# s-will/BiAlign

Hardware: AMD Instinct MI355X
Metric: giga-DP-cells/sec (higher is better)
Workload: dtype int32

## Files before the change

### bialign_amd/csrc/bialign_fill_slim.hpp

```cpp
#pragma once

namespace bialign {

template <int S, int TW, int PPW, bool LEAN = false>
__global__ void __launch_bounds__(64 * TW * PPW, 3) fill_affine_slim_kernel(const DeviceBatch A) {
  static_assert(S >= 1, "packed records need a band");
  using PK_ = Pack<S>;
  using G_ = Geo<S>;
  using R_ = Rec<S, 9, LEAN>;
  constexpr int W = G_::W, R = G_::R, RR = G_::RR, PADB = G_::PADB;
  constexpr int ND = R_::ND, NCH4 = R_::NCH4, TAIL = R_::TAIL, RECDW = R_::RECDW;
  static_assert(R * W < 64, "lane 63 must be free: it is the sentinel source of the exchange");
  extern __shared__ __align__(16) int32_t smem[];

  constexpr int T = TW;
  constexpr int NW = TW * PPW;
  const int L = threadIdx.x & 63;
  const int wv = NW == 1 ? 0 : __builtin_amdgcn_readfirstlane(threadIdx.x >> 6);
  const int pw = wv / TW, w = wv - pw * TW;
  const int slot = blockIdx.x * PPW + pw;
  const bool have_pair = slot < A.launch_pairs;
  const int pid = A.order[have_pair ? slot : 0];
  const PairDesc pd = A.pairs[pid];
  const int n = pd.n, m = pd.m, P = pd.P;
  const int il = L / W, aa = L - il * W;
  const bool live = L < R * W;
  const bool ghost = (il == 0);
  int ringfed_v = (ghost || !live) ? 1 : 0;
  asm volatile("" : "+v"(ringfed_v));
  const bool ringfed = ringfed_v != 0;
  int storing_v;
  {
    const int pad_idx0 = L < W ? L : (L >= R * W ? W + (L - R * W) : 64);
    storing_v = ((live && (LEAN ? il == R - 1 : !ghost)) || (!LEAN && pad_idx0 < R_::SLP - R_::SL)) ? 1 : 0;
  }
  asm volatile("" : "+v"(storing_v));
  const bool storing = storing_v != 0;
  const int beta = A.beta, gamma = A.gamma, delta = A.delta;
  const int k1 = A.k1, k2 = A.k2;
  const int gD = gamma + delta, gg = 2 * gamma, ggdd = 2 * gamma + 2 * delta, dd = 2 * delta;

  using GF = GhostFeed<S, 9, LEAN, 0>;
  constexpr int PERW = GF::RING_DW;
  constexpr int SENTBLK = 4 * GF::NP;
  v4i* ring = reinterpret_cast<v4i*>(smem + wv * GF::RING_DW);
  int32_t* sentblk = smem + NW * PERW;
  volatile int32_t* prog_lds = smem + NW * PERW + SENTBLK + pw * TW;
  const volatile int32_t* const fit_floor = smem + NW * PERW + SENTBLK + FIT_FLOOR_WORD;
  const volatile int32_t* const col0_floor = smem + NW * PERW + SENTBLK + COL0_FLOOR_WORD;
  int32_t* offtab = smem + NW * PERW + SENTBLK + LDS_PROG_WORDS;
  int32_t* s1 = offtab + slim_offtab_dw<S>();
  int32_t* s2 = s1 + k1 * k1;
  uint8_t* codes = reinterpret_cast<uint8_t*>(s2 + k2 * k2);
  const int npad = code_pad(n), mpad = code_pad(m, PADB);
  uint8_t* sa = codes + (size_t)pw * A.slim_code_bytes;
  uint8_t* ca = sa + npad;
  uint8_t* sb = ca + npad;
  uint8_t* cb = sb + mpad;

  for (int t = threadIdx.x; t < NW * PERW + SENTBLK; t += 64 * NW) smem[t] = SENT;
  if (threadIdx.x < LDS_PROG_WORDS) smem[NW * PERW + SENTBLK + threadIdx.x] = prog_word_init(threadIdx.x, A.free_ends);
  if (!LEAN)
    for (int t = threadIdx.x; t < GF::OFFTAB_DW; t += 64 * NW) offtab[t] = (int32_t)GF::lane_offset(t >> 6, t & 63);
  for (int t = threadIdx.x; t < k1 * k1; t += 64 * NW) s1[t] = A.s1[t];
  for (int t = threadIdx.x; t < k2 * k2; t += 64 * NW) s2[t] = A.s2[t];
  if (have_pair) {
    const int tt = threadIdx.x - pw * (64 * TW);
    for (int t = tt; t < n; t += 64 * TW) {
      sa[t] = A.seq_a[pd.seq_a + t];
      ca[t] = A.cls_a[pd.seq_a + t];
    }
    for (int t = tt; t < m + 2 * PADB; t += 64 * TW) {
      const int src = t - PADB;
      const bool ok = src >= 0 && src < m;
      sb[t] = ok ? A.seq_b[pd.seq_b + src] : 0;
      cb[t] = ok ? A.cls_b[pd.seq_b + src] : 0;
    }
  }
  __syncthreads();
  if (!have_pair) return;

  const int addrA = ((L - W) & 63) * 4;
  const int addrB = (live && aa < W - 1 ? ((L - W + 1) & 63) : 63) * 4;
  const bool a_first = (aa == 0);
  const int lane_cap = a_first ? SENT : 0x7fffffff;
  int32_t* const lay = A.layers + pd.layer_off;
  const int64_t pk_bnd_off = (int64_t)pd.G * PK_::RECDW;
  const int rec_last = pd.G - 1;
  const int NSw = (pd.NS - w + T - 1) / T;
  const int H = NSw > 0 ? (NSw - 1) * P + m + G_::MAXOFF + 1 : 0;

  int jj = -(2 * il + aa);
  int strip = 0;
  int rec_base = w * P;
  int i = 0, s1row = 0, s2row = 0;
  bool act_row = false;
  auto set_row = [&](int q) {
    i = (q * T + w) * RR + il - 1;
    const int k = i + aa - S;
    act_row = live && i >= 0 && i <= n && k >= 0 && k <= n;
    s1row = (i >= 1 && i <= n) ? sa[i - 1] * k1 : 0;
    s2row = (k >= 1 && k <= n) ? ca[k - 1] * k2 : 0;
  };
  set_row(0);

  int dA1[2][W], dA2[2][W];
  int dAx[2][W];
  int dB[4][W];
  int dC[2][W];
  int selfv[4][W];
  int pubC[W][8];
  int inC[W][8];
  int inA[W][4], inB[W][8];
#pragma unroll
  for (int bb = 0; bb < W; ++bb) {
    dA1[0][bb] = dA1[1][bb] = dA2[0][bb] = dA2[1][bb] = SENT;
    dAx[0][bb] = dAx[1][bb] = dC[0][bb] = dC[1][bb] = SENT;
#pragma unroll
    for (int x = 0; x < 4; ++x) dB[x][bb] = selfv[x][bb] = inA[bb][x] = SENT;
#pragma unroll
    for (int x = 0; x < 8; ++x) pubC[bb][x] = inB[bb][x] = inC[bb][x] = SENT;
  }
  const uint32_t ring_lds = __builtin_amdgcn_readfirstlane(
      (uint32_t)(uintptr_t)(__attribute__((address_space(3))) int32_t*)smem) + wv * GF::RING_DW * 4;

  using SA = StepAddr<S, LEAN>;
  using GS = GhostSrc<S, LEAN>;
  typedef const __attribute__((address_space(3))) int32_t* lds_cptr;
  typedef __attribute__((address_space(1))) char* gbl_ptr;
  typedef __attribute__((address_space(1))) v4i* gbl_v4i;
  typedef __attribute__((address_space(1))) int32_t* gbl_i32;
  uint32_t st_off = SA::chunk_off(L), st_toff = SA::tail_off(L), gs_fac = GS::factor(L);
  uint32_t gs_lane = GS::lane_byte(L, ring_lds + (NW - wv) * GF::RING_DW * 4);
  asm volatile("" : "+v"(st_off), "+v"(st_toff), "+v"(gs_fac), "+v"(gs_lane));
  int s_ph = 0, s_q = 0;
  int s_adv = 0;
  uint32_t ring_u = 0;
  gbl_ptr sbase = nullptr;

  int blk_q = 0, blk_rem = 0;
  int seen_prog = -0x40000000;
  auto wait_partner = [&](int h_last) __attribute__((always_inline)) {
    if (T == 1) return;
    const int src = w == 0 ? T - 1 : w - 1;
    const int need = h_last + 2 * (R - 1) + 1 - (w == 0 ? P : 0);
    if (seen_prog >= need) return;
    for (int spin = 0; (seen_prog = prog_lds[src]) < need; ++spin) {
      if (spin > A.spin_limit) {
        if (L == 0) atomicOr(A.errflag, 1);
        seen_prog = 0x7fffffff;
        break;
      }
      __builtin_amdgcn_s_sleep(16);
    }
  };
  bool blk_steady = false;
  auto prefetch_block = [&](int h0, int half) __attribute__((always_inline)) {
    wait_partner(h0 + GF::BLK - 1);
    if (!LEAN) blk_steady = GF::steady(blk_q, blk_rem, P, T, w, m, rec_last);
    int Lv = L;
    asm volatile("" : "+v"(Lv));
    if (!LEAN && blk_steady)
      GF::issue_steady(lay, blk_q, blk_rem, P, T, w, offtab, Lv, ring_lds + half * GF::SLOTS * 16);
    else if (LEAN) GF::issue(lay, h0, blk_q, blk_rem, P, T, w, P - 2 * (R - 1), rec_last, Lv, ring_lds + half * GF::SLOTS * 16);
    else GF::issue_packed(lay, pk_bnd_off, m, h0, blk_q, blk_rem, P, T, w, rec_last, Lv, ring_lds + half * GF::SLOTS * 16);
    blk_rem += GF::BLK;
    if (blk_rem >= P) { blk_rem -= P; ++blk_q; }
  };
  prefetch_block(0, 0);
  asm volatile("s_waitcnt vmcnt(0)" ::: "memory");
  int vm_younger = 0;
  int pk_all = 0;
  static_assert(LEAN || PK_::check_in_every_gap(GF::BLK),
                "range check: a test must fall into every non-interior stretch between two strips (pk_all is cleared, not kept, once a row leaves the lattice)");

  auto dmov = [](int& dst, int src) __attribute__((always_inline)) { asm("v_mov_b32 %0, %1" : "=v"(dst) : "v"(src)); };
  auto bperm = [](int addr, int v) __attribute__((always_inline)) -> int { return __builtin_amdgcn_ds_bpermute(addr, v); };

  int mu1n = 0, mu2n[W], sbn = 0, cbn = 0;
  auto lookup_mu = [&]() __attribute__((always_inline)) {
    const int jc = min(max(jj, 0), m + 1);
    mu1n = s1[s1row + sb[jc - 1 + PADB]];
#pragma unroll
    for (int bb = 0; bb < W; ++bb) mu2n[bb] = s2[s2row + cb[jc + bb]];
  };
  auto fetch_codes = [&](auto clamp_tag) __attribute__((always_inline)) {
    const int jc1 = decltype(clamp_tag)::value ? min(max(jj + 1, 0), m + 1) : jj + s_adv + 1;
    sbn = sb[jc1 - 1 + PADB];
    cbn = cb[jc1 + W - 1];
  };
  lookup_mu();
  fetch_codes(BoolTag<true>{});
  int fit_best = SENT, fit_j = 0;

  auto step = [&](auto interior_tag, int g) __attribute__((always_inline)) {
    constexpr bool INTERIOR = decltype(interior_tag)::value;
    if (!INTERIOR) {
      jj += s_adv;
      s_adv = 0;
    }
    const int gt = g & (GF::BLK - 1), ghalf = (g / GF::BLK) & 1;
    if (gt == 0) {
      GF::wait_block(vm_younger);
      if (TW > 1 && L == 0) prog_lds[w] = g - GF::BLK;
      if (!LEAN && (g & (PK_::CHECK - 1)) == 0) {
        const bool bad = live && !ghost && (unsigned)pk_all > 0xffffu;
        if (__builtin_amdgcn_ballot_w64(bad) != 0 && L == 0) atomicOr(A.errflag, 2);
        pk_all = 0;
      }
      if (!LEAN) {
        if (L < GF::BLK * W) {
          bool packed = true;
          if (!blk_steady) {
            int ph = s_ph + L / W, qst = s_q * T + w;
            if (ph >= P) { ph -= P; qst += T; }
            const int ts = ph + 2 * (R - 1), over = ts >= P ? 1 : 0;
            packed = PK_::interior(qst - 1 + over, ts - over * P, m);
          }
          if (packed) {
            v4i* pc = ring + ghalf * GF::SLOTS + L * GF::NP;
            int raw[4 * PK_::NPC], dec[4 * GF::NP];
#pragma unroll
            for (int c = 0; c < PK_::NPC; ++c) {
              const v4i v = pc[c];
              raw[4 * c] = v.x; raw[4 * c + 1] = v.y; raw[4 * c + 2] = v.z; raw[4 * c + 3] = v.w;
            }
#pragma unroll
            for (int d = 0; d < 4 * GF::NP; ++d) {
              const int h = PK_::hw(d < ND ? d : 0);
              const unsigned word = (unsigned)raw[d < ND && d != PK_::ANCHOR ? h >> 1 : 0];
              const unsigned e = d == PK_::ANCHOR ? 0x8000u : PK_::offset_of((h & 1) ? word >> 16 : word & 0xffffu, raw[0]);
              const int v = raw[0] + (int)e;
              dec[d] = d >= ND ? 0 : (pack_corner(W, d % 9, d / 9) ? (e == 0xffffu ? NEG : v) : v);
            }
#pragma unroll
            for (int c = 0; c < GF::NP; ++c) {
              v4i v;
              v.x = dec[4 * c]; v.y = dec[4 * c + 1]; v.z = dec[4 * c + 2]; v.w = dec[4 * c + 3];
              pc[c] = v;
            }
          }
        }
      }
      prefetch_block(g + GF::BLK, ghalf ^ 1);
      vm_younger = 0;
      ring_u = ring_lds + ghalf * GS::HALFB;
      if (A.prio_mode) {
        const int lvl = ((g >> 7) + (wv >> 2)) & 3;
        if (lvl == 0) __builtin_amdgcn_s_setprio(0);
        else if (lvl == 1) __builtin_amdgcn_s_setprio(1);
        else if (lvl == 2) __builtin_amdgcn_s_setprio(2);
        else __builtin_amdgcn_s_setprio(3);
      }
    }
    const int32_t* const gsrc = live ? reinterpret_cast<const int32_t*>(ring + ghalf * GF::SLOTS + (gt * W + aa) * GF::NP)
                                     : sentblk;
    uint32_t gaddr = 0;
    if (INTERIOR) asm("v_mad_u32_u24 %0, %1, %2, %3" : "=v"(gaddr) : "v"(gs_fac), "s"(ring_u), "v"(gs_lane));
    const lds_cptr gsrc_s = (lds_cptr)(uintptr_t)gaddr;
    auto at_store = [](uint32_t& off) __attribute__((always_inline)) -> uint32_t {
      asm volatile("" : "+v"(off));
      return off;
    };

    auto read_dpp = [&](int r) __attribute__((always_inline)) { dpp_from_left<W>(r, inC, pubC, lane_cap); };
    read_dpp(0);

    const int mu1 = mu1n;
    int mu2[W];
#pragma unroll
    for (int bb = 0; bb < W; ++bb) mu2[bb] = mu2n[bb];

    const bool tile_act = INTERIOR ? true : (act_row && jj >= 0 && jj <= m);
    const bool is_origin = INTERIOR ? false : (tile_act && i == 0 && jj == 0 && aa == S);
    const bool row0_diag = INTERIOR ? false : (tile_act && i == 0 && aa == S);
    const bool col0_diag = INTERIOR ? false : (tile_act && jj == 0 && aa == S);
    const int c3M = mu1 + dd, c_Mg = mu1 + gD;

    const int rec = g + rec_base;
    const int pad_idx = L < W ? L : (L >= R * W ? W + (L - R * W) : 64);
    const bool pad_lane = pad_idx < R_::SLP - R_::SL;
    constexpr bool PACKED = INTERIOR && !LEAN;
    const bool do_store = INTERIOR ? storing
                                   : (((live && (LEAN ? il == R - 1 : !ghost)) || (!LEAN && pad_lane)) &&
                                      __builtin_amdgcn_ballot_w64(tile_act && !ghost) != 0 && (TW == 1 || rec <= rec_last));
    const int slot_ = LEAN ? aa : (pad_lane ? R_::SL + pad_idx : L - W);
    if (INTERIOR) vm_younger += PACKED ? PK_::NPC : GF::STORES_PER_STEP;
    else if (__builtin_amdgcn_ballot_w64(do_store) != 0) vm_younger += GF::STORES_PER_STEP;
    int32_t* dst = lay + (int64_t)rec * RECDW;
    if (!INTERIOR && !LEAN) {
      const int tl = jj + 2 * il + aa;
      const int over = tl >= P ? 1 : 0;
      dst = lay + pk_bnd_off + PK_::bidx(strip * T + w + over, tl - over * P, P, m) * RECDW;
    }

    int outv[PACKED ? 1 : ND];
    int pk_base = 0, pk_min = 0, pk_max = 0, pk_e[PACKED ? ND : 1];
    int h2y[3] = {SENT, SENT, SENT};
    int defer[3] = {SENT, SENT, SENT};
#pragma unroll
    for (int bb = 0; bb < W; ++bb) {
      if (bb + 1 < W) read_dpp(bb + 1 < W ? bb + 1 : 0);
      const int l = jj + bb - S;
      const bool act = INTERIOR ? true : (tile_act && l >= 0 && l <= m);
      const int mu2v = mu2[bb];
      const int c_MM = mu1 + mu2v, c_gM = mu2v + gD, c2M = mu2v + dd;

      const AffineCases<W> cases{dA2, bb, dB, dAx, inB, dC, selfv, c_MM, c_Mg, c_gM, gg, ggdd, inC, h2y, c2M, gD, c3M};
      int M[9];
      bool isneg[9] = {};
      if (INTERIOR) {
        if (ringfed) {
#pragma unroll
          for (int q = 0; q < 9; ++q) M[q] = gsrc_s[bb * 9 + q];
        } else {
          int Tv[9];
          cases(Tv);
#pragma unroll
          for (int q = 0; q < 9; ++q) {
            int tv = Tv[q];
            if (can_be_empty<W>(q / 3, q % 3, bb)) {
              isneg[q] = tv < THRESH;
              tv = isneg[q] ? NEG : tv;
            }
            M[q] = tv;
          }
        }
      } else {
        int Gm[9];
#pragma unroll
        for (int q = 0; q < 9; ++q) Gm[q] = SENT;
        if (ghost) {
#pragma unroll
          for (int q = 0; q < 9; ++q) Gm[q] = gsrc[bb * 9 + q];
        }
        int Tv[9];
        cases(Tv);
        const int low = act ? NEG : SENT;
#pragma unroll
        for (int q = 0; q < 9; ++q) {
          const int tv = ghost ? Gm[q] : Tv[q];
          const bool bad = (tv < THRESH) | !act;
          M[q] = bad ? low : tv;
        }
        if (bb == S) M[8] = is_origin ? 0 : M[8];
        if (bb == S && row0_diag) M[8] = imax(M[8], fit_floor[0]);
        if (bb == S && col0_diag) M[8] = imax(M[8], col0_floor[0]);
      }
      if (!PACKED) {
#pragma unroll
        for (int q = 0; q < 9; ++q) outv[PACKED ? 0 : bb * 9 + q] = M[q];
      }
      if (LEAN && bb == S)
        lean_end_rule<INTERIOR>(A, pid, n, m, live && !ghost && aa == S, act_row, i, INTERIOR ? jj + s_adv : jj, fit_best,
                                fit_j, [&] {
          int best = M[0];
#pragma unroll
          for (int q = 1; q < 9; ++q) best = imax(best, M[q]);
          return best;
        });
      if (PACKED) {
        if (bb == 0) {
          pk_base = M[8] - 0x8000;
          pk_min = pk_max = M[8];
        }
        {
          int xs[9];
          int nx = 0;
#pragma unroll
          for (int q = 0; q < 9; ++q) {
            if (bb * 9 + q == PK_::ANCHOR) continue;
            int x = M[q];
            if (pack_corner(W, q, bb)) {
              const bool ng = isneg[q];
              x = ng ? pk_base + 0xffff : x;
            }
            pk_e[PACKED ? bb * 9 + q : 0] = x;
            xs[nx++] = x;
          }
#pragma unroll
          for (int t = 0; t + 1 < nx; t += 2) pk_min = imin(imin(pk_min, xs[t]), xs[t + 1]);
          if (nx & 1) pk_min = imin(pk_min, xs[nx - 1]);
        }
        if (do_store) {
#pragma unroll
          for (int c = 0; c < PK_::NPC; ++c) {
            constexpr int NDWc = PK_::NDW;
            const int dlast = 4 * c + 3 < NDWc - 1 ? 4 * c + 3 : NDWc - 1;
            const int last = PK_::val(2 * dlast + 1);
            if (last >= bb * 9 && last < (bb + 1) * 9) {
              int dw[4];
#pragma unroll
              for (int x = 0; x < 4; ++x) {
                const int d = 4 * c + x;
                const int lo = d < NDWc ? PK_::val(2 * d) : 0, hi = d < NDWc ? PK_::val(2 * d + 1) : 0;
                dw[x] = d == 0 ? pk_base
                               : (d < NDWc ? (int)__builtin_amdgcn_perm((unsigned)pk_e[PACKED ? hi : 0], (unsigned)pk_e[PACKED ? lo : 0], 0x05040100u) : 0);
              }
              if (c < PK_::NCH) {
                v4i v;
                v.x = dw[0]; v.y = dw[1]; v.z = dw[2]; v.w = dw[3];
                *reinterpret_cast<gbl_v4i>(sbase + SA::chunk_imm(c) + at_store(st_off)) = v;
              } else if (slot_ < PK_::TSLOTS) {
                const gbl_i32 tp = reinterpret_cast<gbl_i32>(sbase + SA::TAIL_IMM + at_store(st_toff));
#pragma unroll
                for (int x = 0; x < PK_::TAILDW; ++x) tp[x] = dw[x];
              }
            }
          }
        }
      } else {
        if (do_store) {
#pragma unroll
          for (int c = 0; c < NCH4; ++c) {
            if (4 * c + 3 >= bb * 9 && 4 * c + 3 < (bb + 1) * 9) {
              v4i v;
              v.x = outv[PACKED ? 0 : 4 * c]; v.y = outv[PACKED ? 0 : 4 * c + 1];
              v.z = outv[PACKED ? 0 : 4 * c + 2]; v.w = outv[PACKED ? 0 : 4 * c + 3];
              if (INTERIOR) *reinterpret_cast<gbl_v4i>(sbase + SA::chunk_imm(c) + at_store(st_off)) = v;
              else *reinterpret_cast<v4i*>(dst + c * R_::CH + slot_ * 4) = v;
            }
          }
          if (LEAN && bb == W - 1) {
            const gbl_i32 tp = INTERIOR ? reinterpret_cast<gbl_i32>(sbase + SA::TAIL_IMM + at_store(st_toff)) : nullptr;
#pragma unroll
            for (int t = 0; t < TAIL; ++t) {
              if (INTERIOR) tp[t] = outv[PACKED ? 0 : 4 * NCH4 + t];
              else dst[NCH4 * R_::CH + slot_ * TAIL + t] = outv[PACKED ? 0 : 4 * NCH4 + t];
            }
          }
        }
        if (!LEAN && bb == W - 1) {
          const bool wave_stores = __builtin_amdgcn_ballot_w64(tile_act && !ghost) != 0 && (TW == 1 || rec <= rec_last);
          if (wave_stores) {
            const int tslot = (live && !ghost) ? L - W : R_::SL + (L < W ? L : W + (L - R * W));
#pragma unroll
            for (int t = 0; t < TAIL; ++t) dst[NCH4 * R_::CH + tslot * TAIL + t] = outv[PACKED ? 0 : 4 * NCH4 + t];
          }
        }
      }

      int H2[3][3], H3[3][3], Gd[3][3];
#pragma unroll
      for (int u = 0; u < 3; ++u) {
        H2[u][2] = fM(M[3 * u], M[3 * u + 1], M[3 * u + 2]);
        const int bm = beta + H2[u][2];
        H2[u][0] = imax(M[3 * u], bm);
        H2[u][1] = imax(M[3 * u + 1], bm);
      }
#pragma unroll
      for (int v = 0; v < 3; ++v) {
        H3[2][v] = fM(M[v], M[3 + v], M[6 + v]);
        Gd[2][v] = fM(H2[0][v], H2[1][v], H2[2][v]);
        const int bm3 = beta + H3[2][v], bmg = beta + Gd[2][v];
        H3[0][v] = imax(M[v], bm3);
        H3[1][v] = imax(M[3 + v], bm3);
        Gd[0][v] = imax(H2[0][v], bmg);
        Gd[1][v] = imax(H2[1][v], bmg);
      }
      if (PACKED) {
        pk_max = imax(pk_max, Gd[2][2]);
        if (bb == W - 1) {
          const int acc = pk_all | (pk_max - pk_base + 1) | (pk_min - pk_base);
          pk_all = act_row ? acc : 0;
        }
      }
      pubC[bb][0] = Gd[0][2];
      pubC[bb][1] = Gd[0][1];
#pragma unroll
      for (int u = 0; u < 3; ++u) {
        pubC[bb][2 + u] = H2[u][2];
        pubC[bb][5 + u] = H2[u][1];
      }
      selfv[0][bb] = Gd[0][0];
#pragma unroll
      for (int v = 0; v < 3; ++v) selfv[1 + v][bb] = H3[0][v];
#pragma unroll
      for (int u = 0; u < 3; ++u) h2y[u] = H2[u][0];

      dmov(dA2[0][bb], dA1[0][bb]);
      dmov(dA2[1][bb], dA1[1][bb]);
      dmov(dA1[0][bb], inA[bb][0]);
      dmov(dA1[1][bb], inA[bb][1]);
      dmov(dB[0][bb], inB[bb][0]);
#pragma unroll
      for (int v = 0; v < 3; ++v) dmov(dB[1 + v][bb], inB[bb][2 + v]);
      dC[0][bb] = inC[bb][0];
      dC[1][bb] = inC[bb][1];
      inA[bb][0] = bperm(addrA, Gd[2][2]);
      inA[bb][1] = bperm(addrA, Gd[2][1]);
      inB[bb][0] = bperm(addrB, Gd[2][0]);
#pragma unroll
      for (int v = 0; v < 3; ++v) {
        inB[bb][2 + v] = bperm(addrB, H3[2][v]);
        inB[bb][5 + v] = bperm(addrB, H3[1][v]);
      }
      if (bb >= 1) {
        dmov(dAx[0][bb >= 1 ? bb - 1 : 0], inA[bb >= 1 ? bb - 1 : 0][2]);
        dmov(dAx[1][bb >= 1 ? bb - 1 : 0], inA[bb >= 1 ? bb - 1 : 0][3]);
        inA[bb >= 1 ? bb - 1 : 0][2] = bperm(addrA, defer[0]);
        inA[bb >= 1 ? bb - 1 : 0][3] = bperm(addrA, defer[1]);
        inB[bb >= 1 ? bb - 1 : 0][1] = bperm(addrB, defer[2]);
      }
      defer[0] = Gd[1][2];
      defer[1] = Gd[1][1];
      defer[2] = Gd[1][0];
    }
    dmov(dAx[0][W - 1], inA[W - 1][2]);
    dmov(dAx[1][W - 1], inA[W - 1][3]);
    inA[W - 1][2] = bperm(addrA, defer[0]);
    inA[W - 1][3] = bperm(addrA, defer[1]);
    inB[W - 1][1] = bperm(addrB, defer[2]);

    if (INTERIOR) ++s_adv;
    else ++jj;
    if (!INTERIOR && jj == P) {
      jj = 0;
      ++strip;
      rec_base += (T - 1) * P;
      set_row(strip);
    }
    ++s_ph;
    if (!INTERIOR && s_ph == P) {
      s_ph = 0;
      ++s_q;
    }
    ring_u += GS::STEPB;
    if (INTERIOR) {
      sbase += SA::RECB;
    } else {
      const uint64_t b = (uint64_t)(uintptr_t)(reinterpret_cast<char*>(lay) + SA::record_byte(g + 1, s_q, T, w, P));
      sbase = reinterpret_cast<gbl_ptr>((uintptr_t)((uint64_t)__builtin_amdgcn_readfirstlane((uint32_t)(b >> 32)) << 32 |
                                                    (uint32_t)__builtin_amdgcn_readfirstlane((uint32_t)b)));
    }
    if (INTERIOR) {
      mu1n = s1[s1row + sbn];
#pragma unroll
      for (int bb = 0; bb + 1 < W; ++bb) dmov(mu2n[bb], mu2[bb + 1]);
      mu2n[W - 1] = s2[s2row + cbn];
    } else {
      lookup_mu();
    }
    if (INTERIOR) fetch_codes(BoolTag<false>{});
    else fetch_codes(BoolTag<true>{});
  };

  auto all_interior = [&]() __attribute__((always_inline)) {
    (void)jj, (void)strip;
    return PK_::interior(s_q * T + w, s_ph, m);
  };
  int g = 0;
  while (g < H) {
    while (g < H && !all_interior()) {
      step(BoolTag<false>{}, g);
      ++g;
    }
    while (g < H && all_interior()) {
      step(BoolTag<true>{}, g);
      ++g;
    }
  }
  if (!LEAN && __builtin_amdgcn_ballot_w64(live && !ghost && (unsigned)pk_all > 0xffffu) != 0 && L == 0) atomicOr(A.errflag, 2);
  if (TW > 1) {
    asm volatile("s_waitcnt vmcnt(0)" ::: "memory");
    if (L == 0) prog_lds[w] = 0x7fffffff;
  }
}

}
```

Measured before the change: 215.2.

## Defer A/B lane permutes to next step, holding raw values instead of permuted

Instead of issuing cross-lane permutes for the A and B dependency values right after computing them and keeping the permuted results in registers, the kernel now keeps the raw values (heldA/heldB) and permutes them at the start of the next step, just before they are consumed. This retimes the exchange so fewer permuted in-flight arrays (the old inA array) need to stay live, reducing register pressure and the dmov copies. The trade-off is that permute latency now sits closer to its consumer, which may expose LDS/bpermute latency on the critical path. The dAx[1] source also moves from the deferred path to the held path, which changes the timing of that dependency.

```diff
diff --git a/bialign_amd/csrc/bialign_fill_slim.hpp b/bialign_amd/csrc/bialign_fill_slim.hpp
--- a/bialign_amd/csrc/bialign_fill_slim.hpp
+++ b/bialign_amd/csrc/bialign_fill_slim.hpp
@@ -111,13 +111,17 @@
   int selfv[4][W];
   int pubC[W][8];
   int inC[W][8];
-  int inA[W][4], inB[W][8];
+  int inAx[W];
+  int inB[W][8];
+  int heldA[3][W];
+  int heldB[4][W];
 #pragma unroll
   for (int bb = 0; bb < W; ++bb) {
     dA1[0][bb] = dA1[1][bb] = dA2[0][bb] = dA2[1][bb] = SENT;
     dAx[0][bb] = dAx[1][bb] = dC[0][bb] = dC[1][bb] = SENT;
-#pragma unroll
-    for (int x = 0; x < 4; ++x) dB[x][bb] = selfv[x][bb] = inA[bb][x] = SENT;
+    inAx[bb] = heldA[0][bb] = heldA[1][bb] = heldA[2][bb] = SENT;
+#pragma unroll
+    for (int x = 0; x < 4; ++x) dB[x][bb] = selfv[x][bb] = heldB[x][bb] = SENT;
 #pragma unroll
     for (int x = 0; x < 8; ++x) pubC[bb][x] = inB[bb][x] = inC[bb][x] = SENT;
   }
@@ -297,7 +301,7 @@
     int outv[PACKED ? 1 : ND];
     int pk_base = 0, pk_min = 0, pk_max = 0, pk_e[PACKED ? ND : 1];
     int h2y[3] = {SENT, SENT, SENT};
-    int defer[3] = {SENT, SENT, SENT};
+    int defer[2] = {SENT, SENT};
 #pragma unroll
     for (int bb = 0; bb < W; ++bb) {
       if (bb + 1 < W) read_dpp(bb + 1 < W ? bb + 1 : 0);
@@ -440,6 +444,14 @@
         }
       }
 
+      dmov(dA2[0][bb], dA1[0][bb]);
+      dmov(dA2[1][bb], dA1[1][bb]);
+      dA1[0][bb] = bperm(addrA, heldA[0][bb]);
+      dA1[1][bb] = bperm(addrA, heldA[1][bb]);
+      dAx[1][bb] = bperm(addrA, heldA[2][bb]);
+#pragma unroll
+      for (int x = 0; x < 4; ++x) dB[x][bb] = bperm(addrB, heldB[x][bb]);
+
       int H2[3][3], H3[3][3], Gd[3][3];
 #pragma unroll
       for (int u = 0; u < 3; ++u) {
@@ -478,39 +490,27 @@
 #pragma unroll
       for (int u = 0; u < 3; ++u) h2y[u] = H2[u][0];
 
-      dmov(dA2[0][bb], dA1[0][bb]);
-      dmov(dA2[1][bb], dA1[1][bb]);
-      dmov(dA1[0][bb], inA[bb][0]);
-      dmov(dA1[1][bb], inA[bb][1]);
-      dmov(dB[0][bb], inB[bb][0]);
-#pragma unroll
-      for (int v = 0; v < 3; ++v) dmov(dB[1 + v][bb], inB[bb][2 + v]);
+      heldA[0][bb] = Gd[2][2];
+      heldA[1][bb] = Gd[2][1];
+      heldA[2][bb] = Gd[1][1];
+      heldB[0][bb] = Gd[2][0];
+#pragma unroll
+      for (int v = 0; v < 3; ++v) heldB[1 + v][bb] = H3[2][v];
       dC[0][bb] = inC[bb][0];
       dC[1][bb] = inC[bb][1];
-      inA[bb][0] = bperm(addrA, Gd[2][2]);
-      inA[bb][1] = bperm(addrA, Gd[2][1]);
-      inB[bb][0] = bperm(addrB, Gd[2][0]);
-#pragma unroll
-      for (int v = 0; v < 3; ++v) {
-        inB[bb][2 + v] = bperm(addrB, H3[2][v]);
-        inB[bb][5 + v] = bperm(addrB, H3[1][v]);
-      }
+#pragma unroll
+      for (int v = 0; v < 3; ++v) inB[bb][5 + v] = bperm(addrB, H3[1][v]);
       if (bb >= 1) {
-        dmov(dAx[0][bb >= 1 ? bb - 1 : 0], inA[bb >= 1 ? bb - 1 : 0][2]);
-        dmov(dAx[1][bb >= 1 ? bb - 1 : 0], inA[bb >= 1 ? bb - 1 : 0][3]);
-        inA[bb >= 1 ? bb - 1 : 0][2] = bperm(addrA, defer[0]);
-        inA[bb >= 1 ? bb - 1 : 0][3] = bperm(addrA, defer[1]);
-        inB[bb >= 1 ? bb - 1 : 0][1] = bperm(addrB, defer[2]);
+        dmov(dAx[0][bb >= 1 ? bb - 1 : 0], inAx[bb >= 1 ? bb - 1 : 0]);
+        inAx[bb >= 1 ? bb - 1 : 0] = bperm(addrA, defer[0]);
+        inB[bb >= 1 ? bb - 1 : 0][1] = bperm(addrB, defer[1]);
       }
       defer[0] = Gd[1][2];
-      defer[1] = Gd[1][1];
-      defer[2] = Gd[1][0];
-    }
-    dmov(dAx[0][W - 1], inA[W - 1][2]);
-    dmov(dAx[1][W - 1], inA[W - 1][3]);
-    inA[W - 1][2] = bperm(addrA, defer[0]);
-    inA[W - 1][3] = bperm(addrA, defer[1]);
-    inB[W - 1][1] = bperm(addrB, defer[2]);
+      defer[1] = Gd[1][0];
+    }
+    dmov(dAx[0][W - 1], inAx[W - 1]);
+    inAx[W - 1] = bperm(addrA, defer[0]);
+    inB[W - 1][1] = bperm(addrB, defer[1]);
 
     if (INTERIOR) ++s_adv;
     else ++jj;
```

Measured after the change: 217.3 (median of 6 runs). Within noise of the previous version (+1.0%).
